# near/near-light-client

Hardware: AMD Instinct MI355X
Metric: Sync/Verify proofs/sec at 1/2/4/8 MI355X + achieved HBM GB/s vs roofline (higher is better)
Workload: dtype u64 (Goldilocks field, integer)

## Files before the change

### near-light-client_amd/csrc/gl32.hpp

```cpp
#pragma once
#include "gl.hpp"
#include "poseidon_blocks.inc"

namespace gl32 {

struct F {
    uint32_t lo, hi;
};

__device__ __forceinline__ F from_u64(uint64_t x) { return F{(uint32_t)x, (uint32_t)(x >> 32)}; }
__device__ __forceinline__ uint64_t to_u64(F x) { return ((uint64_t)x.hi << 32) | x.lo; }

__device__ __forceinline__ F add_w2_eps(uint64_t base, uint32_t w2) {
    uint64_t r;
    uint32_t t;
    asm("v_mad_u64_u32 %[r], vcc, %[w2], -1, %[base]\n\t"
        "v_cndmask_b32_e64 %[t], 0, -1, vcc\n\t"
        "v_mad_u64_u32 %[r], vcc, %[t], 1, %[r]"
        : [r] "=&v"(r), [t] "=&v"(t)
        : [w2] "v"(w2), [base] "v"(base)
        : "vcc");
    return from_u64(r);
}

// ... 157 lines not shown
    p[0] = __builtin_amdgcn_perm(t23l, t01l, 0x05040100u);
    p[1] = __builtin_amdgcn_perm(t23l, t01l, 0x07060302u);
    p[2] = __builtin_amdgcn_perm(t23h, t01h, 0x05040100u);
    p[3] = __builtin_amdgcn_perm(t23h, t01h, 0x07060302u);
}
__device__ __forceinline__ uint64_t mad_u64(uint32_t a, uint32_t b, uint64_t c) {
    uint64_t r, sink;
    asm("v_mad_u64_u32 %0, %1, %2, %3, %4" : "=v"(r), "=s"(sink) : "v"(a), "v"(b), "v"(c));
    return r;
}
__device__ __forceinline__ uint64_t mad_u64_sc(uint32_t a, uint32_t b, uint64_t c_uniform) {
    uint64_t r, sink;
    asm("v_mad_u64_u32 %0, %1, %2, %3, %4" : "=v"(r), "=s"(sink) : "v"(a), "v"(b), "s"(c_uniform));
    return r;
}
__device__ __forceinline__ uint64_t mad_u64_one(uint32_t a, uint64_t c) {
    uint64_t r, sink;
    asm("v_mad_u64_u32 %0, %1, %2, 1, %3" : "=v"(r), "=s"(sink) : "v"(a), "v"(c));
    return r;
}
__device__ __forceinline__ F fold_pair(uint64_t t, uint32_t yh, uint32_t k16) {
    uint64_t z, u, sink, sink2;
    asm("v_mad_u64_u32 %0, %1, %2, %3, 0" : "=v"(z), "=s"(sink) : "v"(yh), "v"(k16));
    asm("v_mad_u64_u32 %0, %1, %2, -1, %3" : "=v"(u), "=s"(sink2) : "v"((uint32_t)(z >> 32)), "v"(t));
    uint32_t r1, m;
    asm("v_add_co_u32 %0, vcc, %2, %3\n\t"
        "v_cndmask_b32_e64 %1, 0, -1, vcc"
        : "=v"(r1), "=v"(m)
        : "v"((uint32_t)(u >> 32)), "v"((uint32_t)z)
        : "vcc");
    return from_u64(mad_u64_one(m, ((uint64_t)r1 << 32) | (uint32_t)u));
}

template <int RC>
__device__ __forceinline__ void mds_layer_mfma(F (&s)[12], const i32x4_t a, const uint64_t* __restrict__ rcb) {
    uint32_t k16 = 65536u, bw = MDS_B_BIAS_SLOTS;
    asm("" : "+v"(k16));
    asm("" : "+v"(bw));
    i32x16_t zero;
#pragma unroll
    for (int i = 0; i < 16; i++) zero[i] = 0;
    uint32_t x[2][12], y[2][12];
#pragma unroll
    for (int half = 0; half < 2; half++) {
        uint32_t pl[4][3];
#pragma unroll
        for (int q = 0; q < 3; q++) {
            uint32_t p[4];
            if (half == 0)
                transpose_bytes4(s[4 * q].lo ^ 0x80808080u, s[4 * q + 1].lo ^ 0x80808080u, s[4 * q + 2].lo ^ 0x80808080u,
                                 s[4 * q + 3].lo ^ 0x80808080u, p);
            else
                transpose_bytes4(s[4 * q].hi ^ 0x80808080u, s[4 * q + 1].hi ^ 0x80808080u, s[4 * q + 2].hi ^ 0x80808080u,
                                 s[4 * q + 3].hi ^ 0x80808080u, p);
#pragma unroll
            for (int b = 0; b < 4; b++) pl[b][q] = p[b];
        }
        i32x16_t d[4];
#pragma unroll
        for (int b = 0; b < 4; b++) {
            i32x4_t bf;
            bf.x = (int)pl[b][0]; bf.y = (int)pl[b][1]; bf.z = (int)pl[b][2]; bf.w = (int)bw;
            d[b] = __builtin_amdgcn_mfma_i32_32x32x32_i8(a, bf, zero, 0, 0, 0);
        }
#pragma unroll
        for (int b = 0; b < 4; b++) keep_whole(d[b]);
#pragma unroll
        for (int r = 0; r < 12; r++) {
            x[half][r] = ((uint32_t)d[1][r] << 8) + (uint32_t)d[0][r];
            y[half][r] = ((uint32_t)d[3][r] << 8) + (uint32_t)d[2][r];
        }
        __builtin_amdgcn_sched_barrier(0);
    }
#pragma unroll
    for (int r = 0; r < 12; r++) {
        if (RC == 2 || (RC == 1 && r == 0)) {
            const uint64_t al = mad_u64_one(x[0][r], mad_u64_sc(y[0][r], k16, rcb[r]));
            const uint64_t ah = mad_u64_one(x[1][r], mad_u64_sc(y[1][r], k16, rcb[12 + r]));
            s[r] = fold_acc(al, ah);
        } else {
            const uint64_t t = mad_u64(y[0][r], k16, ((uint64_t)x[1][r] << 32) | x[0][r]);
            s[r] = fold_pair(t, y[1][r], k16);
        }
    }
}

struct BlockOperands {
    i32x4_t a[3];
    i32x16_t seed;
};

template <int G>
__device__ __forceinline__ uint64_t mad_u64_imm(uint32_t a, uint64_t c) {
    uint64_t r, sink;
    asm("v_mad_u64_u32 %0, %1, %2, %3, %4" : "=v"(r), "=s"(sink) : "v"(a), "n"(G), "v"(c));
    return r;
}
__device__ __forceinline__ F fold_pair_x(uint64_t t, uint32_t yh, uint32_t x2, uint32_t k16) {
    uint64_t z, u, sink, sink2;
    asm("v_mad_u64_u32 %0, %1, %2, %3, 0" : "=v"(z), "=s"(sink) : "v"(yh), "v"(k16));
    const uint32_t e = (uint32_t)(z >> 32) + x2;
    asm("v_mad_u64_u32 %0, %1, %2, -1, %3" : "=v"(u), "=s"(sink2) : "v"(e), "v"(t));
    uint32_t r1, m;
    asm("v_add_co_u32 %0, vcc, %2, %3\n\t"
        "v_cndmask_b32_e64 %1, 0, -1, vcc"
        : "=v"(r1), "=v"(m)
        : "v"((uint32_t)(u >> 32)), "v"((uint32_t)z)
        : "vcc");
    return from_u64(mad_u64_one(m, ((uint64_t)r1 << 32) | (uint32_t)u));
// ... 113 lines not shown
```

### near-light-client_amd/csrc/hash_kernels.hip

```cpp
#include <hip/hip_runtime.h>
#include "poseidon.hpp"
#include "launch.hpp"

namespace nlx {

__global__ __launch_bounds__(256, 4) void k_permute_batch(uint64_t* __restrict__ states, size_t n) {
    const size_t t_raw = (size_t)blockIdx.x * blockDim.x + threadIdx.x;
    const bool live = t_raw < n;
    const size_t t = live ? t_raw : n - 1;
    uint64_t s[12];
    const ulonglong2* src = reinterpret_cast<const ulonglong2*>(states + t * 12);
#pragma unroll
    for (int i = 0; i < 6; i++) {
        ulonglong2 v = src[i];
        s[2 * i] = v.x;
        s[2 * i + 1] = v.y;
    }
    poseidon::permute(s);
    if (!live) return;
    ulonglong2* dst = reinterpret_cast<ulonglong2*>(states + t * 12);
#pragma unroll
    for (int i = 0; i < 6; i++) dst[i] = make_ulonglong2(s[2 * i], s[2 * i + 1]);
}

__device__ __forceinline__ void store_digest(uint64_t* __restrict__ out, size_t idx, const uint64_t (&s)[12]) {
    ulonglong2* dst = reinterpret_cast<ulonglong2*>(out + idx * 4);
    dst[0] = make_ulonglong2(gl::canon(s[0]), gl::canon(s[1]));
    dst[1] = make_ulonglong2(gl::canon(s[2]), gl::canon(s[3]));
}

__global__ __launch_bounds__(256, 4) void k_hash_leaves_rowmajor(const uint64_t* __restrict__ rows, uint32_t row_len,
                                                              size_t n_rows, uint64_t* __restrict__ digests) {
    const size_t row_raw = (size_t)blockIdx.x * blockDim.x + threadIdx.x;
    const bool live = row_raw < n_rows;
    const size_t row = live ? row_raw : n_rows - 1;
    uint64_t s[12];
#pragma unroll
    for (int i = 0; i < 12; i++) s[i] = 0;
    const uint64_t* p = rows + row * (size_t)row_len;
    if (row_len <= 4) {
        for (uint32_t c = 0; c < row_len; c++) {
            uint64_t v = p[c];
            if (c == 0) s[0] = v; else if (c == 1) s[1] = v; else if (c == 2) s[2] = v; else s[3] = v;
        }
        if (live) store_digest(digests, row, s);
        return;
    }
#pragma unroll 1
    for (uint32_t c = 0; c < row_len; c += 8) {
        const uint32_t rem = row_len - c;
#pragma unroll
        for (int j = 0; j < 8; j++)
            if ((uint32_t)j < rem) s[j] = p[c + j];
        poseidon::permute_loose(s);
    }
    if (live) store_digest(digests, row, s);
}

__global__ __launch_bounds__(256, 4) void k_merkle_level(const uint64_t* __restrict__ children,
                                                      uint64_t* __restrict__ parents, size_t n_parents, size_t tree_words) {
    children += (size_t)blockIdx.y * tree_words;
    parents += (size_t)blockIdx.y * tree_words;
    const size_t i_raw = (size_t)blockIdx.x * blockDim.x + threadIdx.x;
    const bool live = i_raw < n_parents;
    const size_t i = live ? i_raw : n_parents - 1;
    const ulonglong2* src = reinterpret_cast<const ulonglong2*>(children + i * 8);
    uint64_t s[12];
#pragma unroll
    for (int k = 0; k < 4; k++) {
        ulonglong2 v = src[k];
        s[2 * k] = v.x;
        s[2 * k + 1] = v.y;
    }
    s[8] = s[9] = s[10] = s[11] = 0;
    poseidon::permute_loose(s);
    if (live) store_digest(parents, i, s);
}

constexpr size_t MERKLE_WIDE_MAX_PARENTS = (size_t)1 << 13;
constexpr unsigned MERKLE_FUSED_MAX_LEVELS = 6;
void launch_merkle_fused(hipStream_t st, const uint64_t* children, size_t n_children, unsigned levels, uint32_t n_trees, size_t tree_words);

void launch_permute_batch(hipStream_t st, uint64_t* d_states, size_t n) {
    if (!n) return;
    hipLaunchKernelGGL(k_permute_batch, dim3((unsigned)((n + 255) / 256)), dim3(256), 0, st, d_states, n);
}

void launch_hash_leaves_rowmajor(hipStream_t st, const uint64_t* d_rows, uint32_t row_len, size_t n_rows,
                                 uint64_t* d_digests) {
    if (!n_rows) return;
    hipLaunchKernelGGL(k_hash_leaves_rowmajor, dim3((unsigned)((n_rows + 255) / 256)), dim3(256), 0, st, d_rows,
                       row_len, n_rows, d_digests);
}

const uint64_t* launch_merkle_levels(hipStream_t st, uint64_t* d_digests, size_t n_leaves, unsigned cap_height, uint32_t n_trees, size_t tree_words) {
    size_t cap = (size_t)1 << cap_height;
    uint64_t* cur = d_digests;
    size_t lvl = n_leaves;
    while (lvl > cap) {
        uint64_t* nxt = cur + lvl * 4;
        size_t half = lvl >> 1;
        if (half * n_trees <= MERKLE_WIDE_MAX_PARENTS) {
            unsigned K = 0;
            while (K < MERKLE_FUSED_MAX_LEVELS && (lvl >> K) > cap) K++;
            launch_merkle_fused(st, cur, lvl, K, n_trees, tree_words);
            for (unsigned s = 0; s < K; s++) {
                cur += lvl * 4;
                lvl >>= 1;
// ... 15 lines not shown

__global__ __launch_bounds__(256, 4) void k_hash_lde_leaves(const uint64_t* __restrict__ lde, size_t col_stride,
                                                         uint32_t n_cols, unsigned log_n, unsigned rate_bits,
                                                         uint64_t* __restrict__ digests, uint32_t batch_cols, size_t tree_words) {
    if (batch_cols) {
        const uint32_t c0 = blockIdx.y * batch_cols;
        lde += (size_t)c0 * col_stride;
        n_cols = n_cols - c0 < batch_cols ? n_cols - c0 : batch_cols;
        digests += (size_t)blockIdx.y * tree_words;
    }
    const size_t pos_raw = (size_t)blockIdx.x * blockDim.x + threadIdx.x;
    const bool live = (pos_raw >> (log_n + rate_bits)) == 0;
    const size_t pos = live ? pos_raw : ((size_t)1 << (log_n + rate_bits)) - 1;
    uint64_t s[12];
#pragma unroll
    for (int i = 0; i < 12; i++) s[i] = 0;
    const uint64_t* p = lde + pos;
    const uint32_t r = (uint32_t)(pos >> log_n), k = (uint32_t)(pos & (((size_t)1 << log_n) - 1));
    const size_t leaf = ((size_t)gl::bitrev32(r, rate_bits) << log_n) + gl::bitrev32(k, log_n);
    if (n_cols <= 4) {
        for (uint32_t c = 0; c < n_cols; c++) {
            uint64_t v = p[(size_t)c * col_stride];
            if (c == 0) s[0] = v; else if (c == 1) s[1] = v; else if (c == 2) s[2] = v; else s[3] = v;
        }
        if (live) store_digest(digests, leaf, s);
        return;
    }
#pragma unroll 1
    for (uint32_t c = 0; c < n_cols; c += 8) {
        const uint32_t rem = n_cols - c;
#pragma unroll
        for (int j = 0; j < 8; j++)
            if ((uint32_t)j < rem) s[j] = p[(size_t)(c + j) * col_stride];
        poseidon::permute_loose(s);
    }
    if (live) store_digest(digests, leaf, s);
}

void launch_hash_lde_leaves_wide(hipStream_t st, const uint64_t* d_lde, size_t col_stride, uint32_t n_cols, unsigned log_n,
                                 unsigned rate_bits, uint64_t* d_digests, uint32_t batch_cols, size_t tree_words);

__global__ __launch_bounds__(256, 4) void k_hash_lde_groups(const uint64_t* __restrict__ lde, size_t col_stride, uint32_t n_cols,
                                                            uint32_t group, unsigned log_L, uint64_t* __restrict__ out) {
    const size_t pos_raw = (size_t)blockIdx.x * blockDim.x + threadIdx.x;
    const bool live = (pos_raw >> log_L) == 0;
    const size_t L = (size_t)1 << log_L, pos = live ? pos_raw : L - 1;
    const uint32_t g = blockIdx.y, c0 = g * group, c1 = c0 + group < n_cols ? c0 + group : n_cols;
    uint64_t s[12];
#pragma unroll
    for (int i = 0; i < 12; i++) s[i] = 0;
    const uint64_t* p = lde + pos;
#pragma unroll 1
    for (uint32_t c = c0; c < c1; c += 8) {
        const uint32_t rem = c1 - c;
#pragma unroll
        for (int j = 0; j < 8; j++)
            if ((uint32_t)j < rem) s[j] = p[(size_t)(c + j) * col_stride];
        poseidon::permute_loose(s);
    }
    if (!live) return;
#pragma unroll
    for (int j = 0; j < 4; j++) out[((size_t)(4 * g + j) << log_L) + pos] = gl::canon(s[j]);
}

void launch_hash_lde_leaves_grouped(hipStream_t st, const uint64_t* d_lde, size_t col_stride, uint32_t n_cols, uint32_t group,
                                    unsigned log_n, unsigned rate_bits, uint64_t* d_group_digests, uint64_t* d_digests) {
    const size_t rows = (size_t)1 << (log_n + rate_bits);
    const uint32_t K = (n_cols + group - 1) / group;
    hipLaunchKernelGGL(k_hash_lde_groups, dim3((unsigned)((rows + 255) / 256), K), dim3(256), 0, st, d_lde, col_stride, n_cols, group,
                       log_n + rate_bits, d_group_digests);
    launch_hash_lde_leaves(st, d_group_digests, rows, 4 * K, log_n, rate_bits, d_digests, 0, 0);
}

void launch_hash_lde_leaves(hipStream_t st, const uint64_t* d_lde, size_t col_stride, uint32_t n_cols,
                            unsigned log_n, unsigned rate_bits, uint64_t* d_digests, uint32_t batch_cols, size_t tree_words) {
    size_t rows = (size_t)1 << (log_n + rate_bits);
    const uint32_t n_batches = batch_cols ? (n_cols + batch_cols - 1) / batch_cols : 1;
    const uint32_t widest = batch_cols && batch_cols < n_cols ? batch_cols : n_cols;
    if (rows * n_batches <= HASH_LEAVES_WIDE_MAX_ROWS && widest > 16) {
        launch_hash_lde_leaves_wide(st, d_lde, col_stride, n_cols, log_n, rate_bits, d_digests, batch_cols, tree_words);
        return;
    }
    hipLaunchKernelGGL(k_hash_lde_leaves, dim3((unsigned)((rows + 255) / 256), n_batches), dim3(256), 0, st, d_lde, col_stride,
                       n_cols, log_n, rate_bits, d_digests, batch_cols, tree_words);
}

}

#include "poseidon_quad.hpp"

namespace nlx {
// ... 123 lines not shown
```

### near-light-client_amd/csrc/poseidon.hpp

```cpp
#pragma once
#include "gl.hpp"
#if defined(__HIP__)
#include "gl32.hpp"
#endif
#include "poseidon_constants.inc"

namespace poseidon {

constexpr int WIDTH = 12;
constexpr int RATE = 8;
constexpr int N_ROUNDS = 30;
constexpr int HALF_FULL = 4;
constexpr int N_PARTIAL = 22;

#if defined(__HIP__)
__constant__ static const uint64_t RC_DEV[360] = NLX_POSEIDON_ROUND_CONSTANTS_INIT;
__constant__ static const uint64_t LAYER_RCB_DEV[31 * 24] = NLX_POSEIDON_LAYER_RCB_INIT;
__constant__ static const uint32_t BLOCK_FRAGMENTS_DEV[NLX_POSEIDON_BLOCK_K * 64 * 4] = NLX_POSEIDON_BLOCK_FRAGMENTS_INIT;
__constant__ static const uint32_t BLOCK_SEED_DEV[16] = NLX_POSEIDON_BLOCK_SEED_INIT;
__constant__ static const uint64_t BLOCK_KAPPA_DEV[NLX_POSEIDON_N_BLOCKS * 2 * NLX_POSEIDON_BLOCK_K] = NLX_POSEIDON_BLOCK_KAPPA_INIT;
static_assert(NLX_POSEIDON_BLOCK_K == 3 && NLX_POSEIDON_BLOCK_DMAX < (1 << 20), "gl32::partial_block3 is written for these");

__device__ __forceinline__ gl32::BlockOperands block_operands(uint32_t lane = threadIdx.x & 63) {
    gl32::BlockOperands op;
// ... 27 lines not shown

GL_HD uint64_t mds_fold(uint64_t al, uint64_t ah) {
    uint64_t l = al + (ah << 32);
    uint64_t h = (ah >> 32) + (l < al ? 1u : 0u);
    uint64_t t1 = (h << 32) - h;
    uint64_t res = l + t1;
    if (res < t1) res += gl::EPS;
    return res;
}
GL_HD void mds_layer(uint64_t (&s)[12]) {
    constexpr uint32_t C[12] = {17, 15, 41, 16, 2, 28, 13, 13, 39, 18, 34, 20};
    uint32_t lo[12], hi[12];
#pragma unroll
    for (int i = 0; i < 12; i++) {
        lo[i] = (uint32_t)s[i];
        hi[i] = (uint32_t)(s[i] >> 32);
    }
#pragma unroll
    for (int r = 0; r < 12; r++) {
        uint64_t al = 0, ah = 0;
#pragma unroll
        for (int i = 0; i < 12; i++) {
            al += (uint64_t)lo[(i + r) % 12] * C[i];
            ah += (uint64_t)hi[(i + r) % 12] * C[i];
        }
        if (r == 0) {
            al += (uint64_t)lo[0] * 8u;
            ah += (uint64_t)hi[0] * 8u;
        }
        s[r] = mds_fold(al, ah);
    }
}

GL_HD void permute_loose(uint64_t (&s)[12]) {
    const uint64_t* rc = rc_table();
#if defined(__HIP_DEVICE_COMPILE__)
#if defined(NLX_DEBUG)
    if (__builtin_amdgcn_read_exec() != ~0ull) __builtin_trap();
#endif
    const uint64_t* rcb = LAYER_RCB_DEV;
    const gl32::i32x4_t a = gl32::mds_a_fragment();
    const gl32::BlockOperands op = block_operands();
    gl32::F t[12];
#pragma unroll
    for (int i = 0; i < 12; i++) t[i] = gl32::add_const(gl32::from_u64(s[i]), rc[i]);
#pragma unroll 1
    for (int r = 0; r < HALF_FULL; r++) {
#pragma unroll
        for (int i = 0; i < 12; i++) t[i] = gl32::sbox7(t[i]);
        gl32::mds_layer_mfma<2>(t, a, rcb + (r + 1) * 24);
    }
#pragma unroll 1
    for (int b = 0; b < NLX_POSEIDON_N_BLOCKS; b++)
        gl32::partial_block3<NLX_POSEIDON_BLOCK_GAMMA21>(t, op, BLOCK_KAPPA_DEV + b * 6);
    t[0] = gl32::sbox7(t[0]);
    gl32::mds_layer_mfma<2>(t, a, rcb + (HALF_FULL + N_PARTIAL) * 24);
#pragma unroll 1
    for (int r = HALF_FULL + N_PARTIAL; r < N_ROUNDS - 1; r++) {
#pragma unroll
        for (int i = 0; i < 12; i++) t[i] = gl32::sbox7(t[i]);
        gl32::mds_layer_mfma<2>(t, a, rcb + (r + 1) * 24);
    }
#pragma unroll
    for (int i = 0; i < 12; i++) t[i] = gl32::sbox7(t[i]);
    gl32::mds_layer_mfma<0>(t, a, rcb);
#pragma unroll
    for (int i = 0; i < 12; i++) s[i] = gl32::to_u64(t[i]);
#else
#pragma unroll 1
    for (int r = 0; r < HALF_FULL; r++) {
        for (int i = 0; i < 12; i++) s[i] = sbox7(gl::add_loose(s[i], rc[r * 12 + i]));
        mds_layer(s);
    }
    for (int r = HALF_FULL; r < HALF_FULL + N_PARTIAL; r++) {
        for (int i = 0; i < 12; i++) s[i] = gl::add_loose(s[i], rc[r * 12 + i]);
        s[0] = sbox7(s[0]);
        mds_layer(s);
    }
    for (int r = HALF_FULL + N_PARTIAL; r < N_ROUNDS; r++) {
        for (int i = 0; i < 12; i++) s[i] = sbox7(gl::add_loose(s[i], rc[r * 12 + i]));
        mds_layer(s);
    }
#endif
}

GL_HD void permute(uint64_t (&s)[12]) {
    permute_loose(s);
#pragma unroll
    for (int i = 0; i < 12; i++) s[i] = gl::canon(s[i]);
}

}
```

### near-light-client_amd/csrc/poseidon_blocks.inc

```
#define NLX_POSEIDON_BLOCK_K 3
#define NLX_POSEIDON_N_BLOCKS 7
#define NLX_POSEIDON_BLOCK_DMAX 570945
#define NLX_POSEIDON_BLOCK_FRAGMENTS_INIT { \
    0xc09161c9u, 0x03a15894u, 0x18c8967fu, 0x00001999u, \
    0x3c58ac18u, 0xb4c80430u, 0x3c70e468u, 0x00001400u, \
    0xb06860c8u, 0x2088f0a0u, 0x70e00038u, 0x00002250u, \
    0xfcae2a96u, 0xced63c88u, 0xe4001832u, 0x0000124eu, \
    0x00000000u, 0x00000000u, 0x00000000u, 0x00000000u, \
    0x00000000u, 0x00000000u, 0x00000000u, 0x00000000u, \
    0x00000000u, 0x00000000u, 0x00000000u, 0x00000000u, \
    0x00000000u, 0x00000000u, 0x00000000u, 0x00000000u, \
    0x682f8f7fu, 0x4d27682cu, 0x68383281u, 0x0000271fu, \
    0x04438703u, 0xe56b3cb4u, 0xb420ce4du, 0x00000d7bu, \
    0xb0e9d9a1u, 0x6b99a8f4u, 0xc888d627u, 0x00000d71u, \
    0xc458e458u, 0x3ca83cf0u, 0x04f03c68u, 0x00001c30u, \
    0x00000000u, 0x00000000u, 0x00000000u, 0x00000000u, \
    0x00000000u, 0x00000000u, 0x00000000u, 0x00000000u, \
    0x00000000u, 0x00000000u, 0x00000000u, 0x00000000u, \
    0x00000000u, 0x00000000u, 0x00000000u, 0x00000000u, \
    0xf0b4bc94u, 0xb4f4f0f0u, 0x30a0882cu, 0x0000022cu, \
    0x94985cc0u, 0x04b0c4f0u, 0x3cb0fc68u, 0x00001068u, \
    0x98a16191u, 0x43e958b4u, 0x5868ae2fu, 0x00002931u, \
    0x5c611d61u, 0x87d9e4bcu, 0xac602a8fu, 0x00000fc9u, \
    0x00000000u, 0x00000000u, 0x00000000u, 0x00000000u, \
// ... 142 lines not shown
    0x00000000u, 0x00000000u, 0x00000000u, 0x00000000u, \
    0x13111313u, 0x12141113u, 0x12111311u, 0x00000000u, \
    0x12111312u, 0x14121114u, 0x12111210u, 0x00000000u, \
    0x11101011u, 0x11111112u, 0x110f1110u, 0x00000000u, \
    0x13111213u, 0x12141213u, 0x12111411u, 0x00000000u, \
    0x00000000u, 0x00000000u, 0x00000000u, 0x00000000u, \
    0x00000000u, 0x00000000u, 0x00000000u, 0x00000000u, \
    0x00000000u, 0x00000000u, 0x00000000u, 0x00000000u, \
    0x00000000u, 0x00000000u, 0x00000000u, 0x00000000u, \
    0x110f1111u, 0x11111012u, 0x1010110fu, 0x00000000u, \
    0x13111312u, 0x13131213u, 0x14111211u, 0x00000000u, \
    0x14111314u, 0x13141214u, 0x12111411u, 0x00000000u, \
    0x12101311u, 0x12121113u, 0x11111210u, 0x00000000u, \
    0x00000000u, 0x00000000u, 0x00000000u, 0x00000000u, \
    0x00000000u, 0x00000000u, 0x00000000u, 0x00000000u, \
    0x00000000u, 0x00000000u, 0x00000000u, 0x00000000u, \
    0x00000000u, 0x00000000u, 0x00000000u, 0x00000000u, \
    0x13121313u, 0x13141315u, 0x14121312u, 0x00000000u, \
    0x14111213u, 0x13141213u, 0x12111311u, 0x00000000u, \
    0x11101111u, 0x11111012u, 0x1110110fu, 0x00000000u, \
    0x12111213u, 0x13131313u, 0x13101211u, 0x00000000u, \
    0x00000000u, 0x00000000u, 0x00000000u, 0x00000000u, \
    0x00000000u, 0x00000000u, 0x00000000u, 0x00000000u, \
    0x00000000u, 0x00000000u, 0x00000000u, 0x00000000u, \
    0x00000000u, 0x00000000u, 0x00000000u, 0x00000000u, \
    0x00000000u, 0x00000000u, 0x00000000u, 0x00000000u, \
    0x00000000u, 0x00000000u, 0x00000000u, 0x00000000u, \
    0x00000000u, 0x00000000u, 0x00000000u, 0x00000000u, \
    0x00000000u, 0x00000000u, 0x00000000u, 0x00000000u }
#define NLX_POSEIDON_BLOCK_SEED_INIT { 268902u, 223253u, 247478u, 247223u, 248753u, 274253u, 242633u, 218663u, 227078u, 251303u, 267368u, 285728u, 0u, 0u, 0u, 0u }
#define NLX_POSEIDON_BLOCK_RHO1_INIT { 25u, 15u, 41u, 16u, 2u, 28u, 13u, 13u, 39u, 18u, 34u, 20u }
#define NLX_POSEIDON_BLOCK_RHO2_INIT { 5017u, 5577u, 3889u, 4968u, 6188u, 4656u, 4977u, 5755u, 4895u, 4430u, 5968u, 4864u }
#define NLX_POSEIDON_BLOCK_GAMMA21 25u
#define NLX_POSEIDON_BLOCK_KAPPA_INIT { \
    0x223428b1ull, 0xbaa67178ull, 0x268d7d8cull, 0x7131aa45ull, 0xde0778d0ull, 0xf1417c86ull, \
    0x93047720ull, 0xffee7dd5ull, 0xb30a65f8ull, 0x7cbfbfb4ull, 0x515c5707ull, 0x27b877daull, \
    0xa969797eull, 0xe3e3c5daull, 0x7282b38dull, 0x18f698ecull, 0x023e55b5ull, 0x1ca2c840ull, \
    0x4819d17full, 0x49c240aaull, 0xa80914c3ull, 0x721f49e3ull, 0x42cd749cull, 0x58c51e0eull, \
    0x522a8a6eull, 0xac6afcfeull, 0x0080dad6ull, 0x908e3933ull, 0x8aeee8e7ull, 0x5d33cef7ull, \
    0x2d9dc335ull, 0x257534e8ull, 0x91a785e9ull, 0x3ce6bd74ull, 0xd8a36f5aull, 0xbcb0d556ull, \
    0x575a82e7ull, 0x08d9fddeull, 0x8a49ea3eull, 0xe5dfcdfcull, 0x730f13d7ull, 0xbbe8a3c4ull }
#define NLX_POSEIDON_LAYER_RCB_INIT { \
    0x0ull, 0x0ull, 0x0ull, 0x0ull, 0x0ull, 0x0ull, 0x0ull, 0x0ull, 0x0ull, 0x0ull, 0x0ull, 0x0ull, 0x0ull, 0x0ull, 0x0ull, 0x0ull, 0x0ull, 0x0ull, 0x0ull, 0x0ull, 0x0ull, 0x0ull, 0x0ull, 0x0ull, \
    0xf722c881ull, 0x41c18e55ull, 0x495dc574ull, 0xef6a0781ull, 0xdc5416ccull, 0x8f30c09cull, 0x0d8f8cfaull, 0xae486f38ull, 0xbfc647fbull, 0x1903ff0bull, 0x969c4be7ull, 0x08cbbbadull, 0x86287821ull, 0x59cd1a8aull, 0xc3b919adull, 0xa484c4c5ull, 0x308bbd23ull, 0x6e4a40c1ull, 0x9a2eedb7ull, 0xe360c6e0ull, 0xd5c7718full, 0xc35eae07ull, 0x849c2656ull, 0xc0572c8cull, \
    0x21de0082ull, 0x959a600dull, 0x06391165ull, 0x32825dafull, 0xe30b2c8aull, 0xfcf8535eull, 0x18c2ad87ull, 0x110b3041ull, 0x6ce0e583ull, 0x589d644eull, 0xdb150d61ull, 0xe9c29633ull, 0xe9fa634aull, 0xf56f6d48ull, 0xf7d713e8ull, 0x8297132bull, 0xad6805e0ull, 0xac51d9f5ull, 0x502ad7dcull, 0x57a1550cull, 0x66bbd30eull, 0x0da2abefull, 0xf061274full, 0x28b8ec3aull, \
    0x7e2b9413ull, 0xfee96586ull, 0xaf82ec1cull, 0x72466352ull, 0xe7e14ca1ull, 0x86a46439ull, 0x11d77b75ull, 0xb9c10733ull, 0xa8043e57ull, 0xe6da8699ull, 0x09ef74bfull, 0xcb2ad631ull, 0x92a756e6ull, 0x70e741ebull, 0x019d5ee2ull, 0x6f6f2ed7ull, 0x7cf416cfull, 0x61df517bull, 0x85dc499bull, 0x4b959b48ull, 0xe8be3e5dull, 0xf5c0bc1dull, 0x40b12cbfull, 0xa637093eull, \
    0x184df408ull, 0x57bf31bbull, 0xa6234346ull, 0xde378d7bull, 0x5d4dea83ull, 0x0344d6a1ull, 0x4a7bf308ull, 0x97279301ull, 0xec024747ull, 0xbb21b1a3ull, 0x1ded0893ull, 0x46a41675ull, 0x3cc3f892ull, 0x2e479dc1ull, 0x6f49de07ull, 0x213ce7beull, 0x5b043134ull, 0xa2de4578ull, 0x7103aaf9ull, 0x5326fc0dull, 0xa9ceb74full, 0x27f8ec88ull, 0xfceb4fdaull, 0xfac6ff13ull, \
    0x00000000ull, 0x00000000ull, 0x00000000ull, 0x00000000ull, 0x00000000ull, 0x00000000ull, 0x00000000ull, 0x00000000ull, 0x00000000ull, 0x00000000ull, 0x00000000ull, 0x00000000ull, 0x00000000ull, 0x00000000ull, 0x00000000ull, 0x00000000ull, 0x00000000ull, 0x00000000ull, 0x00000000ull, 0x00000000ull, 0x00000000ull, 0x00000000ull, 0x00000000ull, 0x00000000ull, \
    0x00000000ull, 0x00000000ull, 0x00000000ull, 0x00000000ull, 0x00000000ull, 0x00000000ull, 0x00000000ull, 0x00000000ull, 0x00000000ull, 0x00000000ull, 0x00000000ull, 0x00000000ull, 0x00000000ull, 0x00000000ull, 0x00000000ull, 0x00000000ull, 0x00000000ull, 0x00000000ull, 0x00000000ull, 0x00000000ull, 0x00000000ull, 0x00000000ull, 0x00000000ull, 0x00000000ull, \
    0x00000000ull, 0x00000000ull, 0x00000000ull, 0x00000000ull, 0x00000000ull, 0x00000000ull, 0x00000000ull, 0x00000000ull, 0x00000000ull, 0x00000000ull, 0x00000000ull, 0x00000000ull, 0x00000000ull, 0x00000000ull, 0x00000000ull, 0x00000000ull, 0x00000000ull, 0x00000000ull, 0x00000000ull, 0x00000000ull, 0x00000000ull, 0x00000000ull, 0x00000000ull, 0x00000000ull, \
    0x00000000ull, 0x00000000ull, 0x00000000ull, 0x00000000ull, 0x00000000ull, 0x00000000ull, 0x00000000ull, 0x00000000ull, 0x00000000ull, 0x00000000ull, 0x00000000ull, 0x00000000ull, 0x00000000ull, 0x00000000ull, 0x00000000ull, 0x00000000ull, 0x00000000ull, 0x00000000ull, 0x00000000ull, 0x00000000ull, 0x00000000ull, 0x00000000ull, 0x00000000ull, 0x00000000ull, \
    0x00000000ull, 0x00000000ull, 0x00000000ull, 0x00000000ull, 0x00000000ull, 0x00000000ull, 0x00000000ull, 0x00000000ull, 0x00000000ull, 0x00000000ull, 0x00000000ull, 0x00000000ull, 0x00000000ull, 0x00000000ull, 0x00000000ull, 0x00000000ull, 0x00000000ull, 0x00000000ull, 0x00000000ull, 0x00000000ull, 0x00000000ull, 0x00000000ull, 0x00000000ull, 0x00000000ull, \
    0x00000000ull, 0x00000000ull, 0x00000000ull, 0x00000000ull, 0x00000000ull, 0x00000000ull, 0x00000000ull, 0x00000000ull, 0x00000000ull, 0x00000000ull, 0x00000000ull, 0x00000000ull, 0x00000000ull, 0x00000000ull, 0x00000000ull, 0x00000000ull, 0x00000000ull, 0x00000000ull, 0x00000000ull, 0x00000000ull, 0x00000000ull, 0x00000000ull, 0x00000000ull, 0x00000000ull, \
    0x00000000ull, 0x00000000ull, 0x00000000ull, 0x00000000ull, 0x00000000ull, 0x00000000ull, 0x00000000ull, 0x00000000ull, 0x00000000ull, 0x00000000ull, 0x00000000ull, 0x00000000ull, 0x00000000ull, 0x00000000ull, 0x00000000ull, 0x00000000ull, 0x00000000ull, 0x00000000ull, 0x00000000ull, 0x00000000ull, 0x00000000ull, 0x00000000ull, 0x00000000ull, 0x00000000ull, \
    0x00000000ull, 0x00000000ull, 0x00000000ull, 0x00000000ull, 0x00000000ull, 0x00000000ull, 0x00000000ull, 0x00000000ull, 0x00000000ull, 0x00000000ull, 0x00000000ull, 0x00000000ull, 0x00000000ull, 0x00000000ull, 0x00000000ull, 0x00000000ull, 0x00000000ull, 0x00000000ull, 0x00000000ull, 0x00000000ull, 0x00000000ull, 0x00000000ull, 0x00000000ull, 0x00000000ull, \
    0x00000000ull, 0x00000000ull, 0x00000000ull, 0x00000000ull, 0x00000000ull, 0x00000000ull, 0x00000000ull, 0x00000000ull, 0x00000000ull, 0x00000000ull, 0x00000000ull, 0x00000000ull, 0x00000000ull, 0x00000000ull, 0x00000000ull, 0x00000000ull, 0x00000000ull, 0x00000000ull, 0x00000000ull, 0x00000000ull, 0x00000000ull, 0x00000000ull, 0x00000000ull, 0x00000000ull, \
    0x00000000ull, 0x00000000ull, 0x00000000ull, 0x00000000ull, 0x00000000ull, 0x00000000ull, 0x00000000ull, 0x00000000ull, 0x00000000ull, 0x00000000ull, 0x00000000ull, 0x00000000ull, 0x00000000ull, 0x00000000ull, 0x00000000ull, 0x00000000ull, 0x00000000ull, 0x00000000ull, 0x00000000ull, 0x00000000ull, 0x00000000ull, 0x00000000ull, 0x00000000ull, 0x00000000ull, \
    0x00000000ull, 0x00000000ull, 0x00000000ull, 0x00000000ull, 0x00000000ull, 0x00000000ull, 0x00000000ull, 0x00000000ull, 0x00000000ull, 0x00000000ull, 0x00000000ull, 0x00000000ull, 0x00000000ull, 0x00000000ull, 0x00000000ull, 0x00000000ull, 0x00000000ull, 0x00000000ull, 0x00000000ull, 0x00000000ull, 0x00000000ull, 0x00000000ull, 0x00000000ull, 0x00000000ull, \
    0x00000000ull, 0x00000000ull, 0x00000000ull, 0x00000000ull, 0x00000000ull, 0x00000000ull, 0x00000000ull, 0x00000000ull, 0x00000000ull, 0x00000000ull, 0x00000000ull, 0x00000000ull, 0x00000000ull, 0x00000000ull, 0x00000000ull, 0x00000000ull, 0x00000000ull, 0x00000000ull, 0x00000000ull, 0x00000000ull, 0x00000000ull, 0x00000000ull, 0x00000000ull, 0x00000000ull, \
    0x00000000ull, 0x00000000ull, 0x00000000ull, 0x00000000ull, 0x00000000ull, 0x00000000ull, 0x00000000ull, 0x00000000ull, 0x00000000ull, 0x00000000ull, 0x00000000ull, 0x00000000ull, 0x00000000ull, 0x00000000ull, 0x00000000ull, 0x00000000ull, 0x00000000ull, 0x00000000ull, 0x00000000ull, 0x00000000ull, 0x00000000ull, 0x00000000ull, 0x00000000ull, 0x00000000ull, \
    0x00000000ull, 0x00000000ull, 0x00000000ull, 0x00000000ull, 0x00000000ull, 0x00000000ull, 0x00000000ull, 0x00000000ull, 0x00000000ull, 0x00000000ull, 0x00000000ull, 0x00000000ull, 0x00000000ull, 0x00000000ull, 0x00000000ull, 0x00000000ull, 0x00000000ull, 0x00000000ull, 0x00000000ull, 0x00000000ull, 0x00000000ull, 0x00000000ull, 0x00000000ull, 0x00000000ull, \
    0x00000000ull, 0x00000000ull, 0x00000000ull, 0x00000000ull, 0x00000000ull, 0x00000000ull, 0x00000000ull, 0x00000000ull, 0x00000000ull, 0x00000000ull, 0x00000000ull, 0x00000000ull, 0x00000000ull, 0x00000000ull, 0x00000000ull, 0x00000000ull, 0x00000000ull, 0x00000000ull, 0x00000000ull, 0x00000000ull, 0x00000000ull, 0x00000000ull, 0x00000000ull, 0x00000000ull, \
    0x00000000ull, 0x00000000ull, 0x00000000ull, 0x00000000ull, 0x00000000ull, 0x00000000ull, 0x00000000ull, 0x00000000ull, 0x00000000ull, 0x00000000ull, 0x00000000ull, 0x00000000ull, 0x00000000ull, 0x00000000ull, 0x00000000ull, 0x00000000ull, 0x00000000ull, 0x00000000ull, 0x00000000ull, 0x00000000ull, 0x00000000ull, 0x00000000ull, 0x00000000ull, 0x00000000ull, \
    0x00000000ull, 0x00000000ull, 0x00000000ull, 0x00000000ull, 0x00000000ull, 0x00000000ull, 0x00000000ull, 0x00000000ull, 0x00000000ull, 0x00000000ull, 0x00000000ull, 0x00000000ull, 0x00000000ull, 0x00000000ull, 0x00000000ull, 0x00000000ull, 0x00000000ull, 0x00000000ull, 0x00000000ull, 0x00000000ull, 0x00000000ull, 0x00000000ull, 0x00000000ull, 0x00000000ull, \
    0x00000000ull, 0x00000000ull, 0x00000000ull, 0x00000000ull, 0x00000000ull, 0x00000000ull, 0x00000000ull, 0x00000000ull, 0x00000000ull, 0x00000000ull, 0x00000000ull, 0x00000000ull, 0x00000000ull, 0x00000000ull, 0x00000000ull, 0x00000000ull, 0x00000000ull, 0x00000000ull, 0x00000000ull, 0x00000000ull, 0x00000000ull, 0x00000000ull, 0x00000000ull, 0x00000000ull, \
    0x00000000ull, 0x00000000ull, 0x00000000ull, 0x00000000ull, 0x00000000ull, 0x00000000ull, 0x00000000ull, 0x00000000ull, 0x00000000ull, 0x00000000ull, 0x00000000ull, 0x00000000ull, 0x00000000ull, 0x00000000ull, 0x00000000ull, 0x00000000ull, 0x00000000ull, 0x00000000ull, 0x00000000ull, 0x00000000ull, 0x00000000ull, 0x00000000ull, 0x00000000ull, 0x00000000ull, \
// ... 8 lines not shown
```

### near-light-client_amd/csrc/prover_kernels.hip

```cpp
#include <hip/hip_runtime.h>
#include "gl.hpp"
#include "gate_acc.hpp"
#include "poseidon.hpp"
#include "poseidon_fast_constants.inc"
#include "prover.hpp"

namespace nlx {

__constant__ static const uint64_t FAST_FIRST[12] = NLX_POSEIDON_FAST_FIRST_RC_INIT;
__constant__ static const uint64_t FAST_RC[22] = NLX_POSEIDON_FAST_RC_INIT;
__constant__ static const uint64_t FAST_VS[22][11] = NLX_POSEIDON_FAST_VS_INIT;
__constant__ static const uint64_t FAST_W[22][11] = NLX_POSEIDON_FAST_W_HATS_INIT;
__constant__ static const uint64_t FAST_INIT[11][11] = NLX_POSEIDON_FAST_INITIAL_MATRIX_INIT;

__device__ __forceinline__ uint64_t root_pow(const uint64_t* __restrict__ half_table, uint32_t e, uint32_t half) {
    return e < half ? half_table[e] : gl::P - half_table[e - half];
}

__global__ __launch_bounds__(256) void k_zs_row_products(ZsParams p) {
    const size_t i = (size_t)blockIdx.x * blockDim.x + threadIdx.x;
    const size_t n = (size_t)1 << p.log_n;
    if (i >= n) return;
    const uint64_t x = root_pow(p.w_n_table, (uint32_t)i, (uint32_t)(n >> 1));
    constexpr int MAXQ = 10;
// ... 1091 lines not shown
        hipLaunchKernelGGL(k_fri_combine, dim3((unsigned)((L + 255) / 256)), dim3(256), 0, st, p);
        return;
    }
    uint32_t cols = 0;
    for (int o = 0; o < FRI_VIEWS; o++) cols += p.n_cols[o];
    const uint32_t per_slice = (cols + slices - 1) / slices;
    hipLaunchKernelGGL(k_fri_combine_partial, dim3((unsigned)((L + 255) / 256), slices), dim3(256), 0, st, p, per_slice, scratch);
    hipLaunchKernelGGL(k_fri_combine_finish, dim3((unsigned)((L + 255) / 256)), dim3(256), 0, st, p, slices, scratch);
}

template <int ARITY_BITS>
__global__ __launch_bounds__(256, 4) void k_fri_leaves(const uint64_t* __restrict__ values, unsigned log_n,
                                                    unsigned rate_bits, uint64_t* __restrict__ digests) {
    constexpr int ARITY = 1 << ARITY_BITS;
    const unsigned log_np = log_n - ARITY_BITS;
    const size_t jp_raw = (size_t)blockIdx.x * blockDim.x + threadIdx.x;
    const bool live = (jp_raw >> (log_np + rate_bits)) == 0;
    const size_t jp = live ? jp_raw : ((size_t)1 << (log_np + rate_bits)) - 1;
    const size_t np = (size_t)1 << log_np, n = (size_t)1 << log_n;
    const uint32_t r = (uint32_t)(jp >> log_np), kp = (uint32_t)(jp & (np - 1));
    const ulonglong2* v = reinterpret_cast<const ulonglong2*>(values) + ((size_t)r * n + kp);
    uint64_t s[12];
#pragma unroll
    for (int i = 0; i < 12; i++) s[i] = 0;
    for (int m0 = 0; m0 < ARITY; m0 += 4) {
#pragma unroll
        for (int t = 0; t < 4; t++) {
            const int m = m0 + t;
            const int mm = (int)(__brev((unsigned)m) >> (32 - ARITY_BITS));
            const ulonglong2 e = v[(size_t)mm * np];
            s[2 * t] = e.x;
            s[2 * t + 1] = e.y;
        }
        poseidon::permute_loose(s);
    }
    if (!live) return;
    const size_t leaf = ((size_t)gl::bitrev32(r, rate_bits) << log_np) + gl::bitrev32(kp, log_np);
    ulonglong2* dst = reinterpret_cast<ulonglong2*>(digests + leaf * 4);
    dst[0] = make_ulonglong2(gl::canon(s[0]), gl::canon(s[1]));
    dst[1] = make_ulonglong2(gl::canon(s[2]), gl::canon(s[3]));
}
void launch_fri_leaves(hipStream_t st, const uint64_t* d_values, unsigned log_n, unsigned rate_bits,
                       unsigned arity_bits, uint64_t* d_digests) {
    const size_t leaves = (size_t)1 << (log_n - arity_bits + rate_bits);
    const unsigned blocks = (unsigned)((leaves + 255) / 256);
    if (arity_bits == 4) hipLaunchKernelGGL(k_fri_leaves<4>, dim3(blocks), dim3(256), 0, st, d_values, log_n, rate_bits, d_digests);
    else if (arity_bits == 3) hipLaunchKernelGGL(k_fri_leaves<3>, dim3(blocks), dim3(256), 0, st, d_values, log_n, rate_bits, d_digests);
    else if (arity_bits == 2) hipLaunchKernelGGL(k_fri_leaves<2>, dim3(blocks), dim3(256), 0, st, d_values, log_n, rate_bits, d_digests);
}

template <int ARITY_BITS>
__global__ __launch_bounds__(256) void k_fri_fold(const uint64_t* __restrict__ values, uint64_t* __restrict__ out,
                                                  unsigned log_n, unsigned rate_bits, uint64_t beta_a, uint64_t beta_b,
                                                  uint64_t shift_inv, const uint64_t* __restrict__ w_L_inv_table,
                                                  const uint64_t* __restrict__ w_A_inv_pows, uint64_t arity_inv) {
    constexpr int ARITY = 1 << ARITY_BITS;
    const unsigned log_np = log_n - ARITY_BITS;
    const unsigned log_L = log_n + rate_bits;
    const size_t jp_raw = (size_t)blockIdx.x * blockDim.x + threadIdx.x;
    const bool live = (jp_raw >> (log_np + rate_bits)) == 0;
    const size_t jp = live ? jp_raw : ((size_t)1 << (log_np + rate_bits)) - 1;
    const size_t np = (size_t)1 << log_np, n = (size_t)1 << log_n;
    const uint32_t r = (uint32_t)(jp >> log_np), kp = (uint32_t)(jp & (np - 1));
    const ulonglong2* v = reinterpret_cast<const ulonglong2*>(values) + ((size_t)r * n + kp);
    gl::Ext a[ARITY];
#pragma unroll
    for (int mm = 0; mm < ARITY; mm++) {
// ... 38 lines not shown
    for (size_t i = 0; i < L; i++) {
        const size_t pos = ((i & ((1u << rate_bits) - 1)) * n) + (i >> rate_bits);
        const gl::Ext v{values[2 * pos], values[2 * pos + 1]};
        acc = gl::add(acc, gl::mul(v, wij));
        wij = gl::mul(wij, wj);
    }
    acc = gl::mul(acc, gl::mul(gl::pow(shift_inv, j), L_inv));
    out[2 * j] = acc.a;
    out[2 * j + 1] = acc.b;
}
void launch_fri_final_coeffs(hipStream_t st, const uint64_t* d_values, unsigned log_n, unsigned rate_bits,
                             uint64_t shift, uint64_t* d_out, uint32_t n_out) {
    const unsigned log_L = log_n + rate_bits;
    hipLaunchKernelGGL(k_fri_final_coeffs, dim3((n_out + 63) / 64), dim3(64), 0, st, d_values, log_n, rate_bits,
                       gl::inv(shift), gl::inv(gl::root_of_unity(log_L)), gl::inv((uint64_t)1 << log_L), d_out, n_out);
}

constexpr uint32_t POW_GRID = 256, POW_BLOCK = 256;
__global__ __launch_bounds__(POW_BLOCK, 4) void k_pow_grind(PowParams p, unsigned long long* __restrict__ best) {
    const uint64_t stride = (uint64_t)POW_GRID * POW_BLOCK;
    const uint64_t gid = (uint64_t)blockIdx.x * POW_BLOCK + threadIdx.x;
    for (uint64_t round = 0; round < p.max_rounds; round++) {
        const uint64_t cand = round * stride + gid;
        const unsigned long long b = __hip_atomic_load(best, __ATOMIC_RELAXED, __HIP_MEMORY_SCOPE_AGENT);
        if (__builtin_amdgcn_readfirstlane((uint32_t)(b < round * stride))) return;
        const bool valid = cand < gl::P;
        if (!__any((int)valid)) return;
        uint64_t s[12];
#pragma unroll
        for (int i = 0; i < 12; i++) s[i] = p.state[i];
#pragma unroll
        for (int i = 0; i < 8; i++)
            if ((uint32_t)i == p.pos) s[i] = cand;
        poseidon::permute(s);
        const uint64_t resp = s[7];
        const unsigned lz = resp ? (unsigned)__clzll((long long)resp) : 64u;
        if (valid && lz >= p.bits) atomicMin(best, (unsigned long long)cand);
    }
}
void launch_pow_grind(hipStream_t st, const PowParams& p, unsigned long long* d_best) {
    (void)hipMemsetAsync(d_best, 0xFF, 8, st);
    hipLaunchKernelGGL(k_pow_grind, dim3(POW_GRID), dim3(POW_BLOCK), 0, st, p, d_best);
}

__global__ void k_fri_gather_leaf(const uint64_t* __restrict__ values, unsigned log_n, unsigned rate_bits,
                                  unsigned arity_bits, const uint64_t* __restrict__ leaf_idx, uint64_t* __restrict__ out,
                                  size_t out_stride_words) {
    const uint32_t q = blockIdx.x;
    const uint32_t m = threadIdx.x;
    const uint32_t arity = 1u << arity_bits;
    if (m >= arity) return;
    const unsigned log_np = log_n - arity_bits;
    const size_t np = (size_t)1 << log_np, n = (size_t)1 << log_n;
    const uint64_t leaf = leaf_idx[q];
    const uint32_t r = gl::bitrev32((uint32_t)(leaf >> log_np), rate_bits);
    const uint32_t kp = gl::bitrev32((uint32_t)(leaf & (np - 1)), log_np);
    const uint32_t mm = gl::bitrev32(m, arity_bits);
    const size_t pos = (size_t)r * n + kp + (size_t)mm * np;
    uint64_t* o = out + (size_t)q * out_stride_words + 2 * m;
    o[0] = values[2 * pos];
    o[1] = values[2 * pos + 1];
}
void launch_fri_gather_leaf(hipStream_t st, const uint64_t* d_values, unsigned log_n, unsigned rate_bits,
                            unsigned arity_bits, const uint64_t* d_leaf_idx, uint32_t n_q, uint64_t* d_out,
                            size_t out_stride_words) {
    hipLaunchKernelGGL(k_fri_gather_leaf, dim3(n_q), dim3(64), 0, st, d_values, log_n, rate_bits, arity_bits,
                       d_leaf_idx, d_out, out_stride_words);
}
// ... 172 lines not shown
```

Baseline: 23.21.

## Skip unused output rows in final Poseidon MDS layer and precompute zero-capacity round

Adds row-mask hints to the Poseidon permutation so the last MDS layer only finalises the state lanes that callers actually read next (digest outputs, the sponge lanes that get overwritten, the PoW lane). When the capacity lanes are known to be zero on the first absorb, it also replaces their first-round constant add and S-box with precomputed literals. Every sponge, Merkle, FRI-leaf and PoW call site passes these hints. The saving is ALU work in a compute-bound hash. The cost is extra template paths, and results are wrong if the masks do not match what callers later read.

```diff
diff --git a/near-light-client_amd/csrc/gl32.hpp b/near-light-client_amd/csrc/gl32.hpp
--- a/near-light-client_amd/csrc/gl32.hpp
+++ b/near-light-client_amd/csrc/gl32.hpp
@@ -213,8 +213,21 @@
     return from_u64(mad_u64_one(m, ((uint64_t)r1 << 32) | (uint32_t)u));
 }
 
-template <int RC>
-__device__ __forceinline__ void mds_layer_mfma(F (&s)[12], const i32x4_t a, const uint64_t* __restrict__ rcb) {
+__device__ __forceinline__ uint32_t unread() {
+    uint32_t v;
+    asm volatile("" : "=v"(v));
+    return v;
+}
+template <uint64_t C>
+__device__ __forceinline__ F literal() {
+    F r;
+    asm volatile("v_mov_b32 %0, %2\n\tv_mov_b32 %1, %3" : "=v"(r.lo), "=v"(r.hi) : "n"((uint32_t)C), "n"((uint32_t)(C >> 32)));
+    return r;
+}
+
+template <int RC, bool SOME_ROWS = false>
+__device__ __forceinline__ void mds_layer_mfma(F (&s)[12], const i32x4_t a, const uint64_t* __restrict__ rcb, const uint32_t rows = 0xFFFu) {
+    static_assert(!SOME_ROWS || RC == 0, "only the last layer leaves rows out");
     uint32_t k16 = 65536u, bw = MDS_B_BIAS_SLOTS;
     asm("" : "+v"(k16));
     asm("" : "+v"(bw));
@@ -248,14 +261,24 @@
         for (int b = 0; b < 4; b++) keep_whole(d[b]);
 #pragma unroll
         for (int r = 0; r < 12; r++) {
-            x[half][r] = ((uint32_t)d[1][r] << 8) + (uint32_t)d[0][r];
-            y[half][r] = ((uint32_t)d[3][r] << 8) + (uint32_t)d[2][r];
+            if (!SOME_ROWS || ((rows >> r) & 1)) {
+                uint32_t xr = ((uint32_t)d[1][r] << 8) + (uint32_t)d[0][r];
+                uint32_t yr = ((uint32_t)d[3][r] << 8) + (uint32_t)d[2][r];
+                if (SOME_ROWS) asm volatile("" : "+v"(xr), "+v"(yr));
+                x[half][r] = xr;
+                y[half][r] = yr;
+            } else {
+                x[half][r] = unread();
+                y[half][r] = unread();
+            }
         }
         __builtin_amdgcn_sched_barrier(0);
     }
 #pragma unroll
     for (int r = 0; r < 12; r++) {
-        if (RC == 2 || (RC == 1 && r == 0)) {
+        if (SOME_ROWS && !((rows >> r) & 1)) {
+            s[r] = F{unread(), unread()};
+        } else if (RC == 2 || (RC == 1 && r == 0)) {
             const uint64_t al = mad_u64_one(x[0][r], mad_u64_sc(y[0][r], k16, rcb[r]));
             const uint64_t ah = mad_u64_one(x[1][r], mad_u64_sc(y[1][r], k16, rcb[12 + r]));
             s[r] = fold_acc(al, ah);
diff --git a/near-light-client_amd/csrc/hash_kernels.hip b/near-light-client_amd/csrc/hash_kernels.hip
--- a/near-light-client_amd/csrc/hash_kernels.hip
+++ b/near-light-client_amd/csrc/hash_kernels.hip
@@ -52,7 +52,7 @@
 #pragma unroll
         for (int j = 0; j < 8; j++)
             if ((uint32_t)j < rem) s[j] = p[c + j];
-        poseidon::permute_loose(s);
+        poseidon::permute_loose(s, poseidon::sponge_rows(rem > 8 ? rem - 8 : 0), c == 0);
     }
     if (live) store_digest(digests, row, s);
 }
@@ -73,7 +73,7 @@
         s[2 * k + 1] = v.y;
     }
     s[8] = s[9] = s[10] = s[11] = 0;
-    poseidon::permute_loose(s);
+    poseidon::permute_loose(s, poseidon::out_rows(0, 4), true);
     if (live) store_digest(parents, i, s);
 }
 
@@ -155,7 +155,7 @@
 #pragma unroll
         for (int j = 0; j < 8; j++)
             if ((uint32_t)j < rem) s[j] = p[(size_t)(c + j) * col_stride];
-        poseidon::permute_loose(s);
+        poseidon::permute_loose(s, poseidon::sponge_rows(rem > 8 ? rem - 8 : 0), c == 0);
     }
     if (live) store_digest(digests, leaf, s);
 }
@@ -179,7 +179,7 @@
 #pragma unroll
         for (int j = 0; j < 8; j++)
             if ((uint32_t)j < rem) s[j] = p[(size_t)(c + j) * col_stride];
-        poseidon::permute_loose(s);
+        poseidon::permute_loose(s, poseidon::sponge_rows(rem > 8 ? rem - 8 : 0), c == c0);
     }
     if (!live) return;
 #pragma unroll
diff --git a/near-light-client_amd/csrc/poseidon.hpp b/near-light-client_amd/csrc/poseidon.hpp
--- a/near-light-client_amd/csrc/poseidon.hpp
+++ b/near-light-client_amd/csrc/poseidon.hpp
@@ -83,7 +83,12 @@
     }
 }
 
-GL_HD void permute_loose(uint64_t (&s)[12]) {
+GL_HD constexpr uint32_t out_rows(uint32_t lo, uint32_t hi) { return ((1u << hi) - 1u) & ~((1u << lo) - 1u); }
+constexpr uint32_t ALL_ROWS = 0xFFFu;
+GL_HD constexpr uint32_t sponge_rows(uint32_t left) { return left == 0 ? out_rows(0, 4) : out_rows(left < 8u ? left : 8u, 12u); }
+
+template <bool HINTS>
+GL_HD void permute_body(uint64_t (&s)[12], uint32_t rows, bool cap_zero) {
     const uint64_t* rc = rc_table();
 #if defined(__HIP_DEVICE_COMPILE__)
 #if defined(NLX_DEBUG)
@@ -92,13 +97,29 @@
     const uint64_t* rcb = LAYER_RCB_DEV;
     const gl32::i32x4_t a = gl32::mds_a_fragment();
     const gl32::BlockOperands op = block_operands();
+    const uint32_t rows_u = HINTS ? (uint32_t)__builtin_amdgcn_readfirstlane((int)rows) : ALL_ROWS;
+    const bool cap0 = HINTS && __builtin_amdgcn_readfirstlane((int)cap_zero) != 0;
+    constexpr uint64_t R0_CAP[4] = NLX_POSEIDON_ROUND0_CAP_SBOX_INIT;
     gl32::F t[12];
 #pragma unroll
-    for (int i = 0; i < 12; i++) t[i] = gl32::add_const(gl32::from_u64(s[i]), rc[i]);
+    for (int i = 0; i < 8; i++) t[i] = gl32::add_const(gl32::from_u64(s[i]), rc[i]);
+    if (cap0) {
+        t[8] = gl32::literal<R0_CAP[0]>();
+        t[9] = gl32::literal<R0_CAP[1]>();
+        t[10] = gl32::literal<R0_CAP[2]>();
+        t[11] = gl32::literal<R0_CAP[3]>();
+    } else {
+#pragma unroll
+        for (int i = 8; i < 12; i++) t[i] = gl32::add_const(gl32::from_u64(s[i]), rc[i]);
+    }
 #pragma unroll 1
     for (int r = 0; r < HALF_FULL; r++) {
 #pragma unroll
-        for (int i = 0; i < 12; i++) t[i] = gl32::sbox7(t[i]);
+        for (int i = 0; i < 8; i++) t[i] = gl32::sbox7(t[i]);
+        if (!(cap0 && r == 0)) {
+#pragma unroll
+            for (int i = 8; i < 12; i++) t[i] = gl32::sbox7(t[i]);
+        }
         gl32::mds_layer_mfma<2>(t, a, rcb + (r + 1) * 24);
     }
 #pragma unroll 1
@@ -114,10 +135,12 @@
     }
 #pragma unroll
     for (int i = 0; i < 12; i++) t[i] = gl32::sbox7(t[i]);
-    gl32::mds_layer_mfma<0>(t, a, rcb);
+    gl32::mds_layer_mfma<0, HINTS>(t, a, rcb, rows_u);
 #pragma unroll
     for (int i = 0; i < 12; i++) s[i] = gl32::to_u64(t[i]);
 #else
+    (void)rows;
+    (void)cap_zero;
 #pragma unroll 1
     for (int r = 0; r < HALF_FULL; r++) {
         for (int i = 0; i < 12; i++) s[i] = sbox7(gl::add_loose(s[i], rc[r * 12 + i]));
@@ -135,6 +158,9 @@
 #endif
 }
 
+GL_HD void permute_loose(uint64_t (&s)[12]) { permute_body<false>(s, ALL_ROWS, false); }
+GL_HD void permute_loose(uint64_t (&s)[12], uint32_t rows, bool cap_zero) { permute_body<true>(s, rows, cap_zero); }
+
 GL_HD void permute(uint64_t (&s)[12]) {
     permute_loose(s);
 #pragma unroll
diff --git a/near-light-client_amd/csrc/poseidon_blocks.inc b/near-light-client_amd/csrc/poseidon_blocks.inc
--- a/near-light-client_amd/csrc/poseidon_blocks.inc
+++ b/near-light-client_amd/csrc/poseidon_blocks.inc
@@ -198,6 +198,7 @@
 #define NLX_POSEIDON_BLOCK_RHO1_INIT { 25u, 15u, 41u, 16u, 2u, 28u, 13u, 13u, 39u, 18u, 34u, 20u }
 #define NLX_POSEIDON_BLOCK_RHO2_INIT { 5017u, 5577u, 3889u, 4968u, 6188u, 4656u, 4977u, 5755u, 4895u, 4430u, 5968u, 4864u }
 #define NLX_POSEIDON_BLOCK_GAMMA21 25u
+#define NLX_POSEIDON_ROUND0_CAP_SBOX_INIT { 0xc70fa963a6d76d43ull, 0x8046358185c6e230ull, 0x6e54c050fb2a6ae5ull, 0xb1742ab4a8c81453ull }
 #define NLX_POSEIDON_BLOCK_KAPPA_INIT { \
     0x223428b1ull, 0xbaa67178ull, 0x268d7d8cull, 0x7131aa45ull, 0xde0778d0ull, 0xf1417c86ull, \
     0x93047720ull, 0xffee7dd5ull, 0xb30a65f8ull, 0x7cbfbfb4ull, 0x515c5707ull, 0x27b877daull, \
diff --git a/near-light-client_amd/csrc/prover_kernels.hip b/near-light-client_amd/csrc/prover_kernels.hip
--- a/near-light-client_amd/csrc/prover_kernels.hip
+++ b/near-light-client_amd/csrc/prover_kernels.hip
@@ -1147,7 +1147,7 @@
             s[2 * t] = e.x;
             s[2 * t + 1] = e.y;
         }
-        poseidon::permute_loose(s);
+        poseidon::permute_loose(s, poseidon::sponge_rows((uint32_t)(2 * (ARITY - m0 - 4))), m0 == 0);
     }
     if (!live) return;
     const size_t leaf = ((size_t)gl::bitrev32(r, rate_bits) << log_np) + gl::bitrev32(kp, log_np);
@@ -1252,8 +1252,8 @@
 #pragma unroll
         for (int i = 0; i < 8; i++)
             if ((uint32_t)i == p.pos) s[i] = cand;
-        poseidon::permute(s);
-        const uint64_t resp = s[7];
+        poseidon::permute_loose(s, poseidon::out_rows(7, 8), false);
+        const uint64_t resp = gl::canon(s[7]);
         const unsigned lz = resp ? (unsigned)__clzll((long long)resp) : 64u;
         if (valid && lz >= p.bits) atomicMin(best, (unsigned long long)cand);
     }
```

Result: no change. 23.26 (median of 4 runs) (+0.2%).
